# google-deepmind/mujoco_warp

Measured on NVIDIA H100. Metric: env-steps/sec (whole box) on humanoid.xml at nworld=8192 per GPU, higher is better.
Workload: dtype f32

## Files before the change

### include/mjb200.h

```cpp
#ifndef MJB200_H
#define MJB200_H

#ifdef __cplusplus
extern "C" {
#endif

typedef struct mjbModel mjbModel;
typedef struct mjbData mjbData;

mjbModel* mjb_model_create(void);
void mjb_model_destroy(mjbModel* m);
int mjb_model_set_int(mjbModel* m, const char* name, int value);
int mjb_model_set_float(mjbModel* m, const char* name, float value);
int mjb_model_set_array(mjbModel* m, const char* name, const void* dev_ptr, int nbatch);
int mjb_model_set_array_batched(mjbModel* m, const char* name, const void* dev_ptr, int nbatch, int batch_stride);
int mjb_model_finalize(mjbModel* m);

mjbData* mjb_data_create(int nworld, int nconmax, int naconmax, int njmax, int njmax_pad, int nv_pad);
void mjb_data_destroy(mjbData* d);
int mjb_data_set_array(mjbData* d, const char* name, void* dev_ptr);
int mjb_data_set_int(mjbData* d, const char* name, int value);
int mjb_data_finalize(mjbData* d, const mjbModel* m);

int mjb_step(const mjbModel* m, mjbData* d, void* stream);
// ... 7 lines not shown
int mjb_collision(const mjbModel* m, mjbData* d, void* stream);
int mjb_make_constraint(const mjbModel* m, mjbData* d, void* stream);
int mjb_fwd_velocity(const mjbModel* m, mjbData* d, void* stream);
int mjb_fwd_actuation(const mjbModel* m, mjbData* d, void* stream);
int mjb_fwd_acceleration(const mjbModel* m, mjbData* d, void* stream);
int mjb_factor_m(const mjbModel* m, mjbData* d, void* stream);
int mjb_com_vel(const mjbModel* m, mjbData* d, void* stream);
int mjb_passive(const mjbModel* m, mjbData* d, void* stream);
int mjb_rne(const mjbModel* m, mjbData* d, void* stream);
int mjb_solve_m(const mjbModel* m, mjbData* d, float* x, const float* y, void* stream);
int mjb_mul_m(const mjbModel* m, mjbData* d, float* res, const float* vec, void* stream);
int mjb_sensor_pos(const mjbModel* m, mjbData* d, void* stream);
int mjb_sensor_vel(const mjbModel* m, mjbData* d, void* stream);
int mjb_sensor_acc(const mjbModel* m, mjbData* d, void* stream);
int mjb_contact_force(const mjbModel* m, mjbData* d, const int* contact_ids, int n, int to_world_frame, float* force, void* stream);
int mjb_rungekutta4(const mjbModel* m, mjbData* d, void* stream);
int mjb_solve(const mjbModel* m, mjbData* d, void* stream);
int mjb_euler(const mjbModel* m, mjbData* d, void* stream);
int mjb_implicit(const mjbModel* m, mjbData* d, void* stream);
int mjb_ctrl_noise(const mjbModel* m, mjbData* d, const float* ctrl_center, int step, float noise_std, float noise_rate, void* stream);

int mjb_step_profile(const mjbModel* m, mjbData* d, void* stream, float* ms_out);

int mjb_last_launch_count(void);
const char* mjb_last_error(void);
const char* mjb_version(void);

#ifdef __cplusplus
}
#endif
#endif
```

### mujoco_warp_b200/__init__.py

```python

from . import scenes
from ._src import mjcf
from ._src._lib import build
from ._src.forward import camlight, collision, com_pos, crb, ctrl_noise, euler, factor_m, forward, fwd_acceleration, fwd_actuation
from ._src.forward import fwd_position, fwd_velocity, kinematics, last_launch_count, make_constraint, solve, step, step_profile, transmission
from ._src.forward import com_vel, contact_force, fwd_kinematics, get_state, implicit, mul_m, passive, rne, rungekutta4, sensor_acc, sensor_pos, sensor_vel, set_state, solve_m, step1, step2
from ._src.io import get_data_into, load_trajectory, make_data, override_model, put_data, put_model, reset_data, reset_data_keyframe
from ._src.trace import event_trace_step, flatten_trace
from ._src.types import BroadphaseFilter, BroadphaseType, ConeType, Constraint, ConstraintState, ConstraintType, Contact, Data
from ._src.types import BiasType, DynType, GainType, State, Statistic, TrnType
from ._src.types import DisableBit, EnableBit, GeomType, IntegratorType, JointType, Model, Option, OverflowType, SolverType

__all__ = [n for n in dir() if not n.startswith("_")]
```

### mujoco_warp_b200/_src/forward.py

```python

from __future__ import annotations

import torch

from . import _lib
from .types import Data, Model


def _call(name: str, m: Model, d: Data):
  if d._model is not m and d._model._handle != m._handle:
    raise ValueError("Data was created for a different Model")
  stream = torch.cuda.current_stream().cuda_stream
  _lib.check(getattr(_lib.lib(), name)(m._handle, d._handle, stream))


def step(m: Model, d: Data):
  _call("mjb_step", m, d)


def forward(m: Model, d: Data):
  _call("mjb_forward", m, d)


def fwd_position(m: Model, d: Data):
# ... 192 lines not shown
    euler(m, d)


def ctrl_noise(m: Model, d: Data, step_index: int, ctrl_center: torch.Tensor | None = None, noise_std: float = 0.01, noise_rate: float = 0.1):
  stream = torch.cuda.current_stream().cuda_stream
  ptr = ctrl_center.data_ptr() if ctrl_center is not None else None
  _lib.check(_lib.lib().mjb_ctrl_noise(m._handle, d._handle, ptr, int(step_index), float(noise_std), float(noise_rate), stream))


def last_launch_count() -> int:
  return int(_lib.lib().mjb_last_launch_count())


KERNEL_NAMES = ("position", "collision", "constraint", "velocity", "solver", "integrate")


def step_profile(m: Model, d: Data):
  import ctypes

  out = (ctypes.c_float * 6)()
  stream = torch.cuda.current_stream().cuda_stream
  _lib.check(_lib.lib().mjb_step_profile(m._handle, d._handle, stream, out))
  return dict(zip(KERNEL_NAMES, [float(x) for x in out]))
```

### mujoco_warp_b200/csrc/capi.cu

```cuda
#include <cstdio>
#include <cstdlib>
#include <algorithm>
#include <cstring>
using std::min;
#include <string>

#include "../../include/mjb200.h"
#include "mjb_types.cuh"

struct mjbModel {
  ModelDev dev;
  bool finalized;
};
struct mjbData {
  DataDev dev;
  bool finalized;
  size_t smem[6];
  cudaStream_t aux[8];
  cudaEvent_t ev_fork, ev_join[8];
  int nsplit;
  cudaStream_t sol_aux[8];
  cudaEvent_t sol_fork[8], sol_join[8];
  cudaStream_t vel_aux[8];
  cudaEvent_t vel_fork[8], vel_join[8];
// ... 126 lines not shown
  if (check(cudaMemset(d->dev.world_conadr, 0, sizeof(int) * (size_t)d->dev.nworld), "memset")) return -1;
  if (check(cudaMemset(d->dev.world_ncon, 0, sizeof(int) * (size_t)d->dev.nworld), "memset")) return -1;
  if (check(cudaMalloc(&d->dev.imp_qacc, sizeof(float) * (size_t)d->dev.nworld * (size_t)(m->dev.nv > 0 ? m->dev.nv : 1)), "cudaMalloc(imp_qacc)")) return -1;
  if (check(cudaMalloc(&d->dev.sol_list, sizeof(int) * 2 * (size_t)d->dev.nworld), "cudaMalloc(sol_list)")) return -1;
  if (check(cudaMalloc(&d->dev.sol_count, sizeof(int) * 16), "cudaMalloc(sol_count)")) return -1;
  if (check(cudaMemset(d->dev.sol_count, 0, sizeof(int) * 16), "memset")) return -1;
  for (int i = 0; i < 8; i++) {
    if (check(cudaStreamCreateWithFlags(&d->sol_aux[i], cudaStreamNonBlocking), "cudaStreamCreate")) return -1;
    if (check(cudaEventCreateWithFlags(&d->sol_fork[i], cudaEventDisableTiming), "cudaEventCreate")) return -1;
    if (check(cudaEventCreateWithFlags(&d->sol_join[i], cudaEventDisableTiming), "cudaEventCreate")) return -1;
  }
  d->dev.sol_stream = d->sol_aux[0]; d->dev.sol_fork = d->sol_fork[0]; d->dev.sol_join = d->sol_join[0];
  for (int i = 0; i < 8; i++) {
    if (check(cudaStreamCreateWithFlags(&d->vel_aux[i], cudaStreamNonBlocking), "cudaStreamCreate")) return -1;
    if (check(cudaEventCreateWithFlags(&d->vel_fork[i], cudaEventDisableTiming), "cudaEventCreate")) return -1;
    if (check(cudaEventCreateWithFlags(&d->vel_join[i], cudaEventDisableTiming), "cudaEventCreate")) return -1;
  }
  {
    const char* e = getenv("MJB_FORK");
    d->fork_velocity = (e ? atoi(e) != 0 : false) && m->dev.neq == 0 && d->dev.nworld >= 1024;
  }
  if (m->dev.integrator == INT_RK4 && !d->rk &&
      check(cudaMalloc(&d->rk, sizeof(float) * (size_t)d->dev.nworld * (size_t)(m->dev.nq + 3 * m->dev.nv + 2 * m->dev.na + 1)), "cudaMalloc(rk)")) return -1;
  d->smem[0] = smem_position(m->dev); d->smem[1] = smem_collision(m->dev, d->dev); d->smem[2] = smem_constraint(m->dev, d->dev);
  d->smem[3] = smem_velocity(m->dev); d->smem[4] = smem_solver(m->dev, d->dev); d->smem[5] = smem_integrate(m->dev);
  static const char* names[6] = {"position", "collision", "constraint", "velocity", "solver", "integrate"};
  for (int i = 0; i < 6; i++)
    if (d->smem[i] > kMaxSmem) {
      char buf[160];
      snprintf(buf, sizeof buf, "%s kernel needs %zu B of shared memory per block (> %zu): model/njmax too large for this version", names[i], d->smem[i], kMaxSmem);
      return fail(buf);
    }
  {
    const char* e = getenv("MJB_SPLIT");
    const int want = e ? atoi(e) : 2;
    if (want >= 2 && d->dev.nworld >= 1024) {
      const int ns = want > 8 ? 8 : want;
      for (int i = 0; i < ns; i++) {
        if (check(cudaStreamCreateWithFlags(&d->aux[i], cudaStreamNonBlocking), "cudaStreamCreate")) return -1;
        if (check(cudaEventCreateWithFlags(&d->ev_join[i], cudaEventDisableTiming), "cudaEventCreate")) return -1;
      }
      if (check(cudaEventCreateWithFlags(&d->ev_fork, cudaEventDisableTiming), "cudaEventCreate")) return -1;
      d->nsplit = ns;
    }
  }
  d->finalized = true;
  return 0;
}
// ... 123 lines not shown
int mjb_step_profile(const mjbModel* m, mjbData* d, void* stream, float* ms_out) {
  MJB_ENTER();
  cudaEvent_t ev[7];
  for (int i = 0; i < 7; i++) if (check(cudaEventCreate(&ev[i]), "cudaEventCreate")) return -1;
  cudaEventRecord(ev[0], s);
  MJB_LAUNCH(launch_position(m->dev, d->dev, STG_KINEMATICS | STG_COM_POS | STG_CAMLIGHT | STG_CRB | STG_TRANSMISSION, s), 1);
  cudaEventRecord(ev[1], s);
  MJB_LAUNCH(reset_contact_counters(d->dev, s), 0);
  MJB_LAUNCH(launch_collision(m->dev, d->dev, s), 1);
  cudaEventRecord(ev[2], s);
  MJB_LAUNCH(launch_constraint(m->dev, d->dev, s), 1);
  cudaEventRecord(ev[3], s);
  MJB_LAUNCH(launch_velocity(m->dev, d->dev, STG_VELOCITY | STG_ACTUATION | STG_ACCELERATION, s), 1);
  cudaEventRecord(ev[4], s);
  MJB_LAUNCH(launch_solver(m->dev, d->dev, s), 1);
  cudaEventRecord(ev[5], s);
  MJB_LAUNCH(launch_integrate(m->dev, d->dev, -1, s), 1);
  cudaEventRecord(ev[6], s);
  if (check(cudaEventSynchronize(ev[6]), "cudaEventSynchronize")) return -1;
  for (int i = 0; i < 6; i++) cudaEventElapsedTime(&ms_out[i], ev[i], ev[i + 1]);
  for (int i = 0; i < 7; i++) cudaEventDestroy(ev[i]);
  return 0;
}
int mjb_ctrl_noise(const mjbModel* m, mjbData* d, const float* ctrl_center, int step, float noise_std, float noise_rate, void* stream) {
  MJB_ENTER();
  MJB_LAUNCH(launch_ctrl_noise(m->dev, d->dev, ctrl_center, step, noise_std, noise_rate, s), 1);
  return 0;
}

}
```

### mujoco_warp_b200/csrc/k_position.cu

```cuda
#include <cstdlib>

#include "mjb_math.cuh"
#include "mjb_team.cuh"
#include "mjb_types.cuh"

namespace {

struct PosLayout {
  int qpos, xpos, xquat, xipos, xanchor, xaxis, scom, cinert, cdof, buf, arena, a_gxmat, total;
};

__host__ __device__ inline int pad4(int n) { return (n + 3) & ~3; }
__host__ __device__ inline PosLayout pos_layout(const ModelDev& m) {
  PosLayout L;
  int o = 0;
  auto take = [&](int n) { int r = o; o += pad4(n); return r; };
  L.xpos = take(3 * m.nbody); L.xquat = take(4 * m.nbody); L.xipos = take(3 * m.nbody);
  L.xanchor = take(3 * m.njnt); L.xaxis = take(3 * m.njnt);
  L.buf = L.xpos;
  if (o < pad4(6 * m.nv)) o = pad4(6 * m.nv);
  L.scom = take(3 * m.nbody); L.cinert = take(10 * m.nbody); L.cdof = take(6 * m.nv);
  L.a_gxmat = pad4(3 * m.ngeom);
  int a = pad4(9 * m.nbody);
  if (L.a_gxmat + pad4(9 * m.ngeom) > a) a = L.a_gxmat + pad4(9 * m.ngeom);
  if (pad4(m.nC) > a) a = pad4(m.nC);
  if (pad4(m.nq) > a) a = pad4(m.nq);
  L.arena = take(a);
  L.qpos = L.arena;
  L.total = o;
  return L;
}

template <int LPW, bool BAT>
__global__ void __launch_bounds__(256)
k_position(const __grid_constant__ ModelDev mp, const __grid_constant__ DataDev d, int mask) {
  extern __shared__ __align__(16) float smem[];
  constexpr int G = 32 / LPW;
  Team<LPW> T;
  T.init(d.w0, d.wn, d.nworld);
  if (T.nvalid <= 0) return;
  MJB_WORLD_MODEL(T.w)
  const int lane = T.lane, sub = T.sub, g = T.g, nval = T.nvalid;
  const bool valid = T.valid;
  const PosLayout L = pos_layout(mp);
  float* S = smem + (size_t)(threadIdx.x >> 5) * ((size_t)L.total * G + 4);
  Stager st;
  st.init(reinterpret_cast<uint64_t*>(S + (size_t)L.total * G), lane);
  const int nb = m.nbody, nj = m.njnt, ng = m.ngeom, nv = m.nv;
#define BLK(f) (S + (size_t)L.f * G)
#define ABLK(off) (S + (size_t)(L.arena + (off)) * G)
#define ROW(blk, n) ((blk) + (size_t)g * (n))
  float *qpos = ROW(BLK(qpos), m.nq), *xpos = ROW(BLK(xpos), 3 * nb), *xquat = ROW(BLK(xquat), 4 * nb), *xipos = ROW(BLK(xipos), 3 * nb),
        *xanchor = ROW(BLK(xanchor), 3 * nj), *xaxis = ROW(BLK(xaxis), 3 * nj), *scom = ROW(BLK(scom), 3 * nb), *cinert = ROW(BLK(cinert), 10 * nb),
        *cdof = ROW(BLK(cdof), 6 * nv);
  float *xmat = ROW(ABLK(0), 9 * nb), *ximat = ROW(ABLK(0), 9 * nb), *gxpos = ROW(ABLK(0), 3 * ng), *gxmat = ROW(ABLK(L.a_gxmat), 9 * ng),
        *buf = ROW(BLK(buf), 6 * nv), *Ms = ROW(ABLK(0), m.nC);
  float* crb = cinert;
  const size_t wg = (size_t)T.wg0;
#define GLOAD(blk, field, n) st.load(blk, d.field + wg * (size_t)(n), nval * (n))
#define GSTORE(field, blk, n) st.store(d.field + wg * (size_t)(n), blk, nval * (n))
  const size_t wb = (size_t)T.w;
  const bool kin = mask & STG_KINEMATICS, com = mask & STG_COM_POS, cam = mask & STG_CAMLIGHT, crbm = mask & STG_CRB;

  if (mask & (STG_KINEMATICS | STG_TRANSMISSION)) GLOAD(BLK(qpos), qpos, m.nq);
  if (!kin && (com || cam)) {
    GLOAD(BLK(xpos), xpos, 3 * nb); GLOAD(BLK(xquat), xquat, 4 * nb); GLOAD(BLK(xipos), xipos, 3 * nb);
    GLOAD(BLK(xanchor), xanchor, 3 * nj); GLOAD(BLK(xaxis), xaxis, 3 * nj);
  }
  if (!com && (cam || crbm)) { GLOAD(BLK(scom), subtree_com, 3 * nb); GLOAD(BLK(cinert), cinert, 10 * nb); GLOAD(BLK(cdof), cdof, 6 * nv); }
  st.load_wait();

  if (kin) {
    if (sub == 0) { xpos[0] = xpos[1] = xpos[2] = 0.f; xquat[0] = 1.f; xquat[1] = xquat[2] = xquat[3] = 0.f; }
    __syncwarp();
#pragma unroll 1
    for (int l = 1; l < m.nlevel; l++) {
#pragma unroll 1
      for (int i = m.level_adr[l] + sub; i < m.level_adr[l + 1]; i += LPW) {
        const int b = m.level_body[i], pid = m.body_parentid[b], jntadr = m.body_jntadr[b], jntnum = m.body_jntnum[b];
// ... 68 lines not shown
      }
    }
  }

  __syncwarp();

  if (kin) {
#pragma unroll 2
    for (int b = sub; b < nb; b += LPW) {
      q4 q = ldq(xquat + 4 * b);
      quat_to_mat(q, xmat + 9 * b);
      st3(xipos + 3 * b, ld3(xpos + 3 * b) + qrot(q, ld3(m.body_ipos + 3 * b)));
    }
#pragma unroll 1
    for (int s = valid ? sub : m.nsite; s < m.nsite; s += LPW) {
      const int b = m.site_bodyid[s];
      q4 q = ldq(xquat + 4 * b);
      float mat[9];
      st3(d.site_xpos + (wb * m.nsite + s) * 3, ld3(xpos + 3 * b) + qrot(q, ld3(m.site_pos + 3 * s)));
      quat_to_mat(qmul(q, ldq(m.site_quat + 4 * s)), mat);
      for (int k = 0; k < 9; k++) d.site_xmat[(wb * m.nsite + s) * 9 + k] = mat[k];
    }
    st.store_fence();
    GSTORE(xpos, BLK(xpos), 3 * nb); GSTORE(xquat, BLK(xquat), 4 * nb); GSTORE(xmat, ABLK(0), 9 * nb); GSTORE(xipos, BLK(xipos), 3 * nb);
    GSTORE(xanchor, BLK(xanchor), 3 * nj); GSTORE(xaxis, BLK(xaxis), 3 * nj);
    st.store_commit();
    if (!com) {
      st.store_wait_read();
#pragma unroll 2
      for (int b = sub; b < nb; b += LPW) quat_to_mat(qmul(ldq(xquat + 4 * b), ldq(m.body_iquat + 4 * b)), ximat + 9 * b);
      st.store_fence();
      GSTORE(ximat, ABLK(0), 9 * nb);
      st.store_commit();
    }
  }
  __syncwarp();

  if (com) {
#pragma unroll 2
    for (int b = sub; b < nb; b += LPW) st3(scom + 3 * b, ld3(xipos + 3 * b) * m.body_mass[b]);
    __syncwarp();
#pragma unroll 1
    for (int l = m.nlevel - 2; l >= 0; l--) {
#pragma unroll 1
      for (int i = m.level_adr[l] + sub; i < m.level_adr[l + 1]; i += LPW) {
        const int b = m.level_body[i];
        v3 acc = ld3(scom + 3 * b);
        for (int c = m.body_childadr[b]; c < m.body_childadr[b + 1]; c++) acc = acc + ld3(scom + 3 * m.body_childid[c]);
        st3(scom + 3 * b, acc);
      }
      __syncwarp();
    }
#pragma unroll 2
    for (int b = sub; b < nb; b += LPW) {
      const float ms = m.body_subtreemass[b];
// ... 26 lines not shown
      int dof = m.jnt_dofadr[j];
      const v3 offset = ld3(scom + 3 * m.body_rootid[b]) - ld3(xanchor + 3 * j);
      if (t == JNT_FREE || t == JNT_BALL) {
        float xm[9];
        quat_to_mat(ldq(xquat + 4 * b), xm);
        if (t == JNT_FREE) {
          for (int k = 0; k < 18; k++) cdof[6 * dof + k] = 0.f;
          cdof[6 * dof + 3] = 1.f; cdof[6 * (dof + 1) + 4] = 1.f; cdof[6 * (dof + 2) + 5] = 1.f;
          dof += 3;
        }
        for (int k = 0; k < 3; k++) {
          v3 col = matcol(xm, k);
          st3(cdof + 6 * (dof + k), col); st3(cdof + 6 * (dof + k) + 3, cross(col, offset));
        }
      } else if (t == JNT_SLIDE) {
        st3(cdof + 6 * dof, mk3(0.f, 0.f, 0.f)); st3(cdof + 6 * dof + 3, ld3(xaxis + 3 * j));
      } else {
        v3 ax = ld3(xaxis + 3 * j);
        st3(cdof + 6 * dof, ax); st3(cdof + 6 * dof + 3, cross(ax, offset));
      }
    }
    st.store_fence();
    GSTORE(subtree_com, BLK(scom), 3 * nb); GSTORE(cinert, BLK(cinert), 10 * nb); GSTORE(cdof, BLK(cdof), 6 * nv);
    if (kin) GSTORE(ximat, ABLK(0), 9 * nb);
    st.store_commit();
  }
  __syncwarp();

  if (mask & STG_CAMLIGHT) {
#pragma unroll 1
    for (int c = valid ? sub : m.ncam; c < m.ncam; c += LPW) {
      const int mode = m.cam_mode[c], b = m.cam_bodyid[c], tb = m.cam_targetbodyid[c];
      const bool is_target = mode == CAM_TARGETBODY || mode == CAM_TARGETBODYCOM;
      v3 p; float mat[9];
      if (mode == CAM_TRACK) {
        for (int k = 0; k < 9; k++) mat[k] = m.cam_mat0[9 * c + k];
        p = ld3(xpos + 3 * b) + ld3(m.cam_pos0 + 3 * c);
      } else if (mode == CAM_TRACKCOM) {
        for (int k = 0; k < 9; k++) mat[k] = m.cam_mat0[9 * c + k];
        p = ld3(scom + 3 * b) + ld3(m.cam_poscom0 + 3 * c);
      } else if (is_target && tb >= 0) {
        q4 q = ldq(xquat + 4 * b);
        p = ld3(xpos + 3 * b) + qrot(q, ld3(m.cam_pos + 3 * c));
        v3 tp = mode == CAM_TARGETBODYCOM ? ld3(scom + 3 * tb) : ld3(xpos + 3 * tb);
        v3 m3 = normalize(p - tp), m1 = normalize(cross(mk3(0.f, 0.f, 1.f), m3)), m2 = normalize(cross(m3, m1));
        mat[0] = m1.x; mat[1] = m2.x; mat[2] = m3.x; mat[3] = m1.y; mat[4] = m2.y; mat[5] = m3.y; mat[6] = m1.z; mat[7] = m2.z; mat[8] = m3.z;
      } else {
// ... 26 lines not shown
      }
      if (norm) dir = normalize(dir);
      st3(d.light_xpos + (wb * m.nlight + l) * 3, p);
      st3(d.light_xdir + (wb * m.nlight + l) * 3, dir);
    }
  }


  if (kin) {
    st.store_wait_read();
#pragma unroll 2
    for (int gi = sub; gi < ng; gi += LPW) {
      const int b = m.geom_bodyid[gi];
      if (m.body_weldid[b] == 0 && (m.nmocap == 0 || m.body_mocapid[m.body_rootid[b]] == -1)) {
        for (int k = 0; k < 3; k++) gxpos[3 * gi + k] = d.geom_xpos[(wb * ng + gi) * 3 + k];
        for (int k = 0; k < 9; k++) gxmat[9 * gi + k] = d.geom_xmat[(wb * ng + gi) * 9 + k];
      } else {
        q4 q = ldq(xquat + 4 * b);
        st3(gxpos + 3 * gi, ld3(xpos + 3 * b) + qrot(q, ld3(m.geom_pos + 3 * gi)));
        quat_to_mat(qmul(q, ldq(m.geom_quat + 4 * gi)), gxmat + 9 * gi);
      }
    }
    st.store_fence();
    GSTORE(geom_xpos, ABLK(0), 3 * ng); GSTORE(geom_xmat, ABLK(L.a_gxmat), 9 * ng);
    st.store_commit();
  }

  if (crbm) {
    st.store_wait_read();
#pragma unroll 1
    for (int l = m.nlevel - 2; l >= 1; l--) {
#pragma unroll 1
      for (int i = m.level_adr[l] + sub; i < m.level_adr[l + 1]; i += LPW) {
        const int b = m.level_body[i];
        float acc[10];
#pragma unroll
        for (int k = 0; k < 10; k++) acc[k] = crb[10 * b + k];
#pragma unroll 1
        for (int c = m.body_childadr[b]; c < m.body_childadr[b + 1]; c++) {
          const float* cc = crb + 10 * m.body_childid[c];
#pragma unroll
          for (int k = 0; k < 10; k++) acc[k] += cc[k];
        }
#pragma unroll
        for (int k = 0; k < 10; k++) crb[10 * b + k] = acc[k];
      }
      __syncwarp();
    }
#pragma unroll 2
    for (int dd = sub; dd < nv; dd += LPW) inert_vec(crb + 10 * m.dof_bodyid[dd], cdof + 6 * dd, buf + 6 * dd);
    __syncwarp();
#pragma unroll 4
    for (int e = sub; e < m.nC; e += LPW) {
      const int i = m.M_entry_row[e], j = m.M_colind[e];
      float v = dot6(cdof + 6 * j, buf + 6 * i);
      if (i == j) v += m.dof_armature[i];
      Ms[e] = v;
    }
    st.store_fence();
    GSTORE(crb, BLK(cinert), 10 * nb); GSTORE(M, ABLK(0), m.nC);
    st.store_commit();
  }
  st.store_wait_read();
#undef GLOAD
#undef GSTORE
#undef BLK
#undef ABLK
#undef ROW
}

}

static TeamShape pos_shape(const ModelDev& m) {
  TeamShape t = team_shape((size_t)pos_layout(m).total, "MJB_LPW_POS", "MJB_WPB_POS");
  if (m.batched && t.lpw != 32) { t = team_shape_fixed((size_t)pos_layout(m).total, 32, 2); }
  return t;
}
size_t smem_position(const ModelDev& m) { return pos_shape(m).block_bytes; }

cudaError_t launch_position(const ModelDev& m, const DataDev& d, int mask, cudaStream_t s) {
  const TeamShape t = pos_shape(m);
  const size_t smem = t.block_bytes;
  const int lpw = t.lpw, G = 32 / lpw, wpb = t.wpb;
  void (*kern)(ModelDev, DataDev, int) = m.batched ? k_position<32, true> : lpw == 4 ? k_position<4, false> : lpw == 8 ? k_position<8, false> : lpw == 16 ? k_position<16, false> : k_position<32, false>;
  static size_t configured[5] = {0, 0, 0, 0, 0};
  const int ki = m.batched ? 4 : lpw == 4 ? 0 : lpw == 8 ? 1 : lpw == 16 ? 2 : 3;
  if (smem > 48 * 1024 && smem > configured[ki]) {
    cudaError_t e = cudaFuncSetAttribute(kern, cudaFuncAttributeMaxDynamicSharedMemorySize, (int)smem);
    if (e != cudaSuccess) return e;
    configured[ki] = smem;
  }
  const int ngroups = (d.wn + G - 1) / G, grid = (ngroups + wpb - 1) / wpb;
  kern<<<grid, 32 * wpb, smem, s>>>(m, d, mask);
  return cudaGetLastError();
}
```

### mujoco_warp_b200/csrc/k_velocity.cu

```cuda
#include <cstdlib>

#include "mjb_math.cuh"
#include "mjb_team.cuh"
#include "mjb_types.cuh"

namespace {

struct VelLayout { int qvel, cdof, cinert, cvel, cdofdot, cacc, cfrc, qpas, qbias, qact, qsm, qld, x, af, total; };
__host__ __device__ inline VelLayout vel_layout(const ModelDev& m) {
  VelLayout L;
  int o = 0;
  auto take = [&](int n) { int r = o; o += (n + 3) & ~3; return r; };
  L.qvel = take(m.nv);
  const int a0 = o;
  L.cdof = take(6 * m.nv); L.cinert = take(10 * m.nbody); L.cvel = take(6 * m.nbody);
  L.cdofdot = take(6 * m.nv); L.cacc = take(6 * m.nbody); L.cfrc = take(6 * m.nbody);
  L.qld = a0;
  if (o - a0 < ((m.qld_total + 3) & ~3)) o = a0 + ((m.qld_total + 3) & ~3);
  L.qpas = take(m.nv); L.qbias = take(m.nv); L.qact = take(m.nv); L.qsm = take(m.nv);
  L.x = L.qpas; L.af = take(m.nu);
  L.total = o;
  return L;
}

template <int LPW>
__device__ __forceinline__ void team_chol_upper(float* U, int n, float* x, bool solve, int sub) {
#pragma unroll 1
  for (int j = 0; j < n; j++) {
    const int iend = solve ? n + 1 : n;
#pragma unroll 1
    for (int i = j + sub; i < iend; i += LPW) {
      const bool rhs = i == n;
      const float* col = rhs ? x : U + i;
      const int cs = rhs ? 1 : n;
      float s0 = rhs ? x[j] : U[j * n + i], s1 = 0.f;
      int k = 0;
#pragma unroll 4
      for (; k + 1 < j; k += 2) {
        s0 -= U[k * n + j] * col[k * cs];
        s1 -= U[(k + 1) * n + j] * col[(k + 1) * cs];
      }
      if (k < j) s0 -= U[k * n + j] * col[k * cs];
      if (rhs) x[j] = s0 + s1; else U[j * n + i] = s0 + s1;
// ... 196 lines not shown
    if (v_all || (mask & STG_RNE)) {
    for (int k = sub; k < 6; k += LPW) cacc[k] = k < 3 ? 0.f : ((m.disableflags & DSBL_GRAVITY) ? 0.f : -(k == 3 ? m.gravity_x : k == 4 ? m.gravity_y : m.gravity_z));
    __syncwarp();
#pragma unroll 1
    for (int l = 1; l < m.nlevel; l++) {
#pragma unroll 1
      for (int i = m.level_adr[l] + sub; i < m.level_adr[l + 1]; i += LPW) {
        const int b = m.level_body[i], pid = m.body_parentid[b];
        float a[6];
#pragma unroll
        for (int k = 0; k < 6; k++) a[k] = cacc[6 * pid + k];
#pragma unroll 1
        for (int q = 0; q < m.body_dofnum[b]; q++) {
          const int dof = m.body_dofadr[b] + q;
          const float v = qvel[dof];
#pragma unroll
          for (int k = 0; k < 6; k++) a[k] += cdofdot[6 * dof + k] * v;
        }
#pragma unroll
        for (int k = 0; k < 6; k++) cacc[6 * b + k] = a[k];
      }
      __syncwarp();
    }
#pragma unroll 2
    for (int b = sub; b < nb; b += LPW) {
      float f[6] = {0.f, 0.f, 0.f, 0.f, 0.f, 0.f};
      if (b > 0) {
        float iv[6], g[6];
        inert_vec(cinert + 10 * b, cacc + 6 * b, f);
        inert_vec(cinert + 10 * b, cvel + 6 * b, iv);
        motion_cross_force(cvel + 6 * b, iv, g);
#pragma unroll
        for (int k = 0; k < 6; k++) f[k] += g[k];
      }
#pragma unroll
      for (int k = 0; k < 6; k++) cfrc[6 * b + k] = f[k];
    }
    __syncwarp();
#pragma unroll 1
    for (int l = m.nlevel - 2; l >= 0; l--) {
#pragma unroll 1
      for (int i = m.level_adr[l] + sub; i < m.level_adr[l + 1]; i += LPW) {
        const int b = m.level_body[i];
        float acc[6];
#pragma unroll
        for (int k = 0; k < 6; k++) acc[k] = cfrc[6 * b + k];
// ... 134 lines not shown
#pragma unroll
      for (int k = 0; k < MREG; k++) {
        const int e = sub + k * LPW;
        if (e >= e0 && e < e1) U[(m.M_colind[e] - start) * n + (m.M_entry_row[e] - start)] = mreg[k];
      }
#pragma unroll 1
      for (int e = max(e0, MREG * LPW) + ((sub - max(e0, MREG * LPW)) % LPW + LPW) % LPW; e < e1; e += LPW)
        U[(m.M_colind[e] - start) * n + (m.M_entry_row[e] - start)] = Mw[e];
      __syncwarp();
      team_chol_upper<LPW>(U, n, x + start, acc, sub);
    }
    st.store_fence();
    if (acc) { GSTORE(qfrc_smooth, qsm, nv); GSTORE(qacc_smooth, x, nv); }
    GSTORE(qLD, qld, m.qld_total);
    st.store_commit();
  }
  st.store_wait_read();
#undef GLOAD
#undef GSTORE
}

}

static TeamShape vel_shape(const ModelDev& m) {
  TeamShape t = team_shape((size_t)vel_layout(m).total, "MJB_LPW_VEL", "MJB_WPB_VEL");
  if (m.batched && t.lpw != 32) t = team_shape_fixed((size_t)vel_layout(m).total, 32, 2);
  return t;
}
size_t smem_velocity(const ModelDev& m) { return vel_shape(m).block_bytes; }

template <bool PEXT>
static void (*vel_kernel(int lpw, bool bat))(ModelDev, DataDev, int) {
  if (bat) return k_velocity<PEXT, 32, true>;
  return lpw == 4 ? k_velocity<PEXT, 4, false> : lpw == 8 ? k_velocity<PEXT, 8, false> : lpw == 16 ? k_velocity<PEXT, 16, false> : k_velocity<PEXT, 32, false>;
}

cudaError_t launch_velocity(const ModelDev& m, const DataDev& d, int mask, cudaStream_t s) {
  const TeamShape t = vel_shape(m);
  const size_t smem = t.block_bytes;
  static size_t configured[2][5] = {{0, 0, 0, 0, 0}, {0, 0, 0, 0, 0}};
  const int ext = (m.has_gravcomp || m.ntendon > 0) ? 1 : 0;
  const int lpw = t.lpw, G = 32 / lpw, wpb = t.wpb, ki = m.batched ? 4 : lpw == 4 ? 0 : lpw == 8 ? 1 : lpw == 16 ? 2 : 3;
  void (*kern)(ModelDev, DataDev, int) = ext ? vel_kernel<true>(lpw, m.batched) : vel_kernel<false>(lpw, m.batched);
  if (smem > 48 * 1024 && smem > configured[ext][ki]) {
    cudaError_t e = cudaFuncSetAttribute(kern, cudaFuncAttributeMaxDynamicSharedMemorySize, (int)smem);
    if (e != cudaSuccess) return e;
    configured[ext][ki] = smem;
  }
  const int ngroups = (d.wn + G - 1) / G, grid = (ngroups + wpb - 1) / wpb;
  kern<<<grid, 32 * wpb, smem, s>>>(m, d, mask);
  return cudaGetLastError();
}
```

### mujoco_warp_b200/csrc/mjb_team.cuh

```cuda
#pragma once
#include <cstdint>
#include <cstdlib>
#include <cuda_runtime.h>

#include "mjb_math.cuh"

template <int LPW>
__device__ __forceinline__ float team_sum(float v) {
#pragma unroll
  for (int o = LPW / 2; o > 0; o >>= 1) v += __shfl_xor_sync(FULL_MASK, v, o);
  return v;
}
template <int LPW>
__device__ __forceinline__ int team_sum_i(int v) {
#pragma unroll
  for (int o = LPW / 2; o > 0; o >>= 1) v += __shfl_xor_sync(FULL_MASK, v, o);
  return v;
}
template <int LPW>
__device__ __forceinline__ bool team_any(bool p, int g) {
  const unsigned b = __ballot_sync(FULL_MASK, p);
  return LPW == 32 ? b != 0u : ((b >> (g * LPW)) & ((1u << (LPW & 31)) - 1u)) != 0u;
}

// ... 43 lines not shown
    asm volatile("fence.proxy.async.shared::cta;" ::: "memory");
    __syncwarp();
  }
  __device__ __forceinline__ void store(float* g, const float* s, int n) {
    if (bulk_ok(g, s, n)) {
      if (lane == 0) {
        asm volatile("cp.async.bulk.global.shared::cta.bulk_group [%0], [%1], %2;" ::"l"(g), "r"(smem_u32(s)), "r"((uint32_t)n * 4u) : "memory");
        pending_store = true;
      }
    } else {
#pragma unroll 1
      for (int i = lane; i < n; i += 32) g[i] = s[i];
    }
  }
  __device__ __forceinline__ void store_commit() {
    if (lane == 0 && pending_store) asm volatile("cp.async.bulk.commit_group;" ::: "memory");
  }
  __device__ __forceinline__ void store_wait_read() {
    if (lane == 0 && pending_store) { asm volatile("cp.async.bulk.wait_group.read 0;" ::: "memory"); pending_store = false; }
    __syncwarp();
  }
};

struct TeamShape { int lpw, wpb; size_t warp_bytes, block_bytes; };
inline TeamShape team_shape(size_t world_words, const char* env_lpw, const char* env_wpb) {
  constexpr size_t kBlockMax = 200 * 1024;
  auto bytes = [&](int lpw) { return (world_words * (size_t)(32 / lpw) + 4) * sizeof(float); };
  const char* e = getenv(env_lpw);
  int lpw = e ? atoi(e) : 8;
  if (lpw != 4 && lpw != 8 && lpw != 16 && lpw != 32) lpw = 8;
  while (lpw < 32 && bytes(lpw) > kBlockMax / 2) lpw *= 2;
  e = getenv(env_wpb);
  int wpb = e ? atoi(e) : 2;
  if (wpb < 1) wpb = 1;
  if (wpb > 8) wpb = 8;
  while (wpb > 1 && bytes(lpw) * wpb > kBlockMax) wpb--;
  TeamShape t;
  t.lpw = lpw; t.wpb = wpb; t.warp_bytes = bytes(lpw); t.block_bytes = t.warp_bytes * wpb;
  return t;
}

inline TeamShape team_shape_fixed(size_t world_words, int lpw, int wpb) {
  TeamShape t;
  t.lpw = lpw; t.wpb = wpb; t.warp_bytes = (world_words * (size_t)(32 / lpw) + 4) * sizeof(float);
  while (t.wpb > 1 && t.warp_bytes * t.wpb > 200 * 1024) t.wpb--;
  t.block_bytes = t.warp_bytes * t.wpb;
  return t;
}

template <int LPW>
struct Team {
  static constexpr int G = 32 / LPW;
  int lane, sub, g;
  int wg0, nvalid;
  int w;
  bool valid;
// ... 10 lines not shown
```

### mujoco_warp_b200/csrc/mjb_types.cuh

```cuda
#pragma once
#include <cuda_runtime.h>

#define MJB_MODEL_INTS(X) \
  X(nq) X(nv) X(nu) X(nbody) X(njnt) X(ngeom) X(nsite) X(ncam) X(nlight) X(nC) X(ntree) X(nJmom) X(nlevel) \
  X(nxn_npair) X(nlimit) X(nfricdof) X(nmaxpyramid) X(integrator) X(cone) X(solver) X(iterations) \
  X(ls_iterations) X(disableflags) X(enableflags) X(broadphase) X(broadphase_filter) X(qld_total) X(maxtree) X(has_multicontact_geom) X(neq) X(nlimit_ball) X(has_gravcomp) X(nmocap) X(npair) X(has_convex_pair) X(ccd_iterations) X(epa_iterations) X(nsensor) X(nsensordata) X(sensor_subtree_vel) X(sensor_rne_postconstraint) X(nmesh) X(na) X(ntendon) X(nJten) X(ntenfric) X(nwrap)
#define MJB_MODEL_FLOATS(X) \
  X(timestep) X(tolerance) X(ls_tolerance) X(impratio_invsqrt) X(meaninertia) X(gravity_x) X(gravity_y) X(gravity_z) X(ccd_tolerance)
#define MJB_MODEL_IARRS(X) \
  X(body_parentid) X(body_rootid) X(body_weldid) X(body_mocapid) X(body_jntnum) X(body_jntadr) X(body_dofnum) X(body_dofadr) \
  X(body_childadr) X(body_childid) X(level_adr) X(level_body) \
  X(jnt_type) X(jnt_qposadr) X(jnt_dofadr) X(jnt_bodyid) X(jnt_actfrclimited) X(jnt_actgravcomp) X(jnt_limited_adr) \
  X(dof_bodyid) X(dof_jntid) X(dof_parentid) X(dof_fricloss_adr) X(M_rownnz) X(M_rowadr) X(M_colind) X(M_entry_row) X(mulm_rowadr) X(mulm_col) X(mulm_madr) \
  X(tree_dofadr) X(tree_dofnum) X(tree_qLDadr) \
  X(geom_type) X(geom_condim) X(geom_bodyid) X(geom_priority) \
  X(actuator_trnid) X(actuator_gaintype) X(actuator_biastype) X(actuator_ctrllimited) X(actuator_forcelimited) \
  X(actuator_dyntype) X(actuator_actadr) X(actuator_actnum) X(actuator_actlimited) X(actuator_actearly) X(actuator_trntype) \
  X(ten_J_rownnz) X(ten_J_rowadr) X(ten_J_colind) X(tendon_adr) X(tendon_num) X(wrap_objid) X(tendon_limited) X(tendon_actfrclimited) \
  X(moment_rownnz0) X(moment_rowadr0) X(moment_colind0) X(dofact_adr) X(dofact_act) X(dofact_mom) \
  X(cam_mode) X(cam_bodyid) X(cam_targetbodyid) X(light_mode) X(light_bodyid) X(light_targetbodyid) X(site_bodyid) \
  X(nxn_geom_pair) X(nxn_pairid) X(body_isdofancestor) X(eq_type) X(eq_obj1id) X(eq_obj2id) X(jnt_limited_ball_adr) X(pair_dim) \
  X(sensor_type) X(sensor_datatype) X(sensor_needstage) X(sensor_objtype) X(sensor_objid) X(sensor_reftype) X(sensor_refid) X(sensor_dim) X(sensor_adr) X(site_type) \
  X(geom_dataid) X(mesh_vertadr) X(mesh_vertnum) X(mesh_graphadr) X(mesh_graph) X(mesh_polynum) X(mesh_polyadr) X(mesh_polyvertadr) X(mesh_polyvertnum) \
  X(mesh_polyvert) X(mesh_polymapadr) X(mesh_polymapnum) X(mesh_polymap)
// ... 117 lines not shown
       STG_COMVEL = 16, STG_PASSIVE = 32, STG_RNE = 64 };

constexpr int MJB_WARPS_PER_BLOCK = 1;

cudaError_t launch_position(const ModelDev& m, const DataDev& d, int stage_mask, cudaStream_t s);
cudaError_t launch_collision(const ModelDev& m, const DataDev& d, cudaStream_t s);
cudaError_t launch_collision_mesh(const ModelDev& m, const DataDev& d, cudaStream_t s);
size_t smem_collision_mesh(const ModelDev& m, const DataDev& d);
cudaError_t reset_contact_counters(const DataDev& d, cudaStream_t s);
cudaError_t launch_constraint(const ModelDev& m, const DataDev& d, cudaStream_t s);
cudaError_t launch_efc_csr(const ModelDev& m, const DataDev& d, cudaStream_t s);
cudaError_t launch_velocity(const ModelDev& m, const DataDev& d, int stage_mask, cudaStream_t s);
cudaError_t launch_solve_m(const ModelDev& m, const DataDev& d, float* x, const float* y, cudaStream_t s);
cudaError_t launch_mul_m(const ModelDev& m, const DataDev& d, float* res, const float* vec, cudaStream_t s);
cudaError_t launch_solver(const ModelDev& m, const DataDev& d, cudaStream_t s);
int solver_launch_count(const ModelDev& m, const DataDev& d);
cudaError_t launch_integrate(const ModelDev& m, const DataDev& d, int integrator, cudaStream_t s);
cudaError_t launch_implicit_solve(const ModelDev& m, const DataDev& d, float* qacc_out, cudaStream_t s);
size_t smem_implicit(const ModelDev& m);
cudaError_t launch_sensor(const ModelDev& m, const DataDev& d, int stages, cudaStream_t s);
cudaError_t launch_contact_force(const ModelDev& m, const DataDev& d, const int* contact_ids, int n, int to_world, float* out, cudaStream_t s);
cudaError_t launch_rk_stage(const ModelDev& m, const DataDev& d, float* rk, int stage, cudaStream_t s);
cudaError_t launch_ctrl_noise(const ModelDev& m, const DataDev& d, const float* ctrl_center, int step, float std, float rate, cudaStream_t s);
size_t smem_position(const ModelDev& m);
size_t smem_collision(const ModelDev& m, const DataDev& d);
size_t smem_constraint(const ModelDev& m, const DataDev& d);
size_t smem_velocity(const ModelDev& m);
size_t smem_solver(const ModelDev& m, const DataDev& d);
size_t smem_integrate(const ModelDev& m);
```

Before: 19.41 million.

## Shrink position/velocity smem layouts and pick warps-per-block from occupancy model

Repacks the shared-memory layouts of the position and velocity kernels so more buffers alias each other, which shrinks the per-world footprint. Warps-per-block is now chosen automatically by modelling SM residency from shared memory, register and block limits against nworld, and the shared-memory carveout is set explicitly. The goal is more worlds resident per SM and fewer launch waves. Adds a residency query API and an extra store_wait_read to protect against the new aliasing, at the risk of hazards if any aliased buffer is still live.

After: 20.80 million (median of 6 runs). +7.2%, better.

```diff
diff --git a/include/mjb200.h b/include/mjb200.h
--- a/include/mjb200.h
+++ b/include/mjb200.h
@@ -53,6 +53,8 @@
 
 int mjb_step_profile(const mjbModel* m, mjbData* d, void* stream, float* ms_out);
 
+int mjb_team_residency(const mjbModel* m, const mjbData* d, int* position_worlds, int* velocity_worlds);
+
 int mjb_last_launch_count(void);
 const char* mjb_last_error(void);
 const char* mjb_version(void);
diff --git a/mujoco_warp_b200/__init__.py b/mujoco_warp_b200/__init__.py
--- a/mujoco_warp_b200/__init__.py
+++ b/mujoco_warp_b200/__init__.py
@@ -3,7 +3,7 @@
 from ._src import mjcf
 from ._src._lib import build
 from ._src.forward import camlight, collision, com_pos, crb, ctrl_noise, euler, factor_m, forward, fwd_acceleration, fwd_actuation
-from ._src.forward import fwd_position, fwd_velocity, kinematics, last_launch_count, make_constraint, solve, step, step_profile, transmission
+from ._src.forward import fwd_position, fwd_velocity, kinematics, last_launch_count, make_constraint, solve, step, step_profile, team_residency, transmission
 from ._src.forward import com_vel, contact_force, fwd_kinematics, get_state, implicit, mul_m, passive, rne, rungekutta4, sensor_acc, sensor_pos, sensor_vel, set_state, solve_m, step1, step2
 from ._src.io import get_data_into, load_trajectory, make_data, override_model, put_data, put_model, reset_data, reset_data_keyframe
 from ._src.trace import event_trace_step, flatten_trace
diff --git a/mujoco_warp_b200/_src/forward.py b/mujoco_warp_b200/_src/forward.py
--- a/mujoco_warp_b200/_src/forward.py
+++ b/mujoco_warp_b200/_src/forward.py
@@ -238,3 +238,13 @@
   stream = torch.cuda.current_stream().cuda_stream
   _lib.check(_lib.lib().mjb_step_profile(m._handle, d._handle, stream, out))
   return dict(zip(KERNEL_NAMES, [float(x) for x in out]))
+
+
+def team_residency(m: Model, d: Data):
+  import ctypes
+
+  f = _lib.lib().mjb_team_residency
+  f.argtypes = [ctypes.c_void_p, ctypes.c_void_p, ctypes.POINTER(ctypes.c_int), ctypes.POINTER(ctypes.c_int)]
+  pos, vel = ctypes.c_int(), ctypes.c_int()
+  _lib.check(f(m._handle, d._handle, ctypes.byref(pos), ctypes.byref(vel)))
+  return {"position": pos.value, "velocity": vel.value}
diff --git a/mujoco_warp_b200/csrc/capi.cu b/mujoco_warp_b200/csrc/capi.cu
--- a/mujoco_warp_b200/csrc/capi.cu
+++ b/mujoco_warp_b200/csrc/capi.cu
@@ -172,8 +172,8 @@
   }
   if (m->dev.integrator == INT_RK4 && !d->rk &&
       check(cudaMalloc(&d->rk, sizeof(float) * (size_t)d->dev.nworld * (size_t)(m->dev.nq + 3 * m->dev.nv + 2 * m->dev.na + 1)), "cudaMalloc(rk)")) return -1;
-  d->smem[0] = smem_position(m->dev); d->smem[1] = smem_collision(m->dev, d->dev); d->smem[2] = smem_constraint(m->dev, d->dev);
-  d->smem[3] = smem_velocity(m->dev); d->smem[4] = smem_solver(m->dev, d->dev); d->smem[5] = smem_integrate(m->dev);
+  d->smem[0] = smem_position(m->dev, d->dev); d->smem[1] = smem_collision(m->dev, d->dev); d->smem[2] = smem_constraint(m->dev, d->dev);
+  d->smem[3] = smem_velocity(m->dev, d->dev); d->smem[4] = smem_solver(m->dev, d->dev); d->smem[5] = smem_integrate(m->dev);
   static const char* names[6] = {"position", "collision", "constraint", "velocity", "solver", "integrate"};
   for (int i = 0; i < 6; i++)
     if (d->smem[i] > kMaxSmem) {
@@ -343,6 +343,13 @@
   for (int i = 0; i < 7; i++) cudaEventDestroy(ev[i]);
   return 0;
 }
+int mjb_team_residency(const mjbModel* m, const mjbData* d, int* position_worlds, int* velocity_worlds) {
+  if (!m || !d || !m->finalized || !d->finalized) return fail("model/data not finalized");
+  if (!position_worlds || !velocity_worlds) return fail("mjb_team_residency: null output");
+  if (check(resident_worlds_position(m->dev, d->dev, position_worlds), "resident_worlds_position")) return -1;
+  if (check(resident_worlds_velocity(m->dev, d->dev, velocity_worlds), "resident_worlds_velocity")) return -1;
+  return 0;
+}
 int mjb_ctrl_noise(const mjbModel* m, mjbData* d, const float* ctrl_center, int step, float noise_std, float noise_rate, void* stream) {
   MJB_ENTER();
   MJB_LAUNCH(launch_ctrl_noise(m->dev, d->dev, ctrl_center, step, noise_std, noise_rate, s), 1);
diff --git a/mujoco_warp_b200/csrc/k_position.cu b/mujoco_warp_b200/csrc/k_position.cu
--- a/mujoco_warp_b200/csrc/k_position.cu
+++ b/mujoco_warp_b200/csrc/k_position.cu
@@ -7,7 +7,7 @@
 namespace {
 
 struct PosLayout {
-  int qpos, xpos, xquat, xipos, xanchor, xaxis, scom, cinert, cdof, buf, arena, a_gxmat, total;
+  int qpos, xpos, xquat, xipos, xanchor, xaxis, scom, cinert, cdof, buf, arena, gxpos, gxmat, M, total;
 };
 
 __host__ __device__ inline int pad4(int n) { return (n + 3) & ~3; }
@@ -16,17 +16,14 @@
   int o = 0;
   auto take = [&](int n) { int r = o; o += pad4(n); return r; };
   L.xpos = take(3 * m.nbody); L.xquat = take(4 * m.nbody); L.xipos = take(3 * m.nbody);
-  L.xanchor = take(3 * m.njnt); L.xaxis = take(3 * m.njnt);
-  L.buf = L.xpos;
-  if (o < pad4(6 * m.nv)) o = pad4(6 * m.nv);
-  L.scom = take(3 * m.nbody); L.cinert = take(10 * m.nbody); L.cdof = take(6 * m.nv);
-  L.a_gxmat = pad4(3 * m.ngeom);
-  int a = pad4(9 * m.nbody);
-  if (L.a_gxmat + pad4(9 * m.ngeom) > a) a = L.a_gxmat + pad4(9 * m.ngeom);
-  if (pad4(m.nC) > a) a = pad4(m.nC);
-  if (pad4(m.nq) > a) a = pad4(m.nq);
-  L.arena = take(a);
+  L.xanchor = take(3 * m.njnt); L.xaxis = take(3 * m.njnt); L.scom = take(3 * m.nbody);
+  L.arena = take(pad4(m.nq) > pad4(9 * m.nbody) ? m.nq : 9 * m.nbody);
   L.qpos = L.arena;
+  L.gxpos = L.xipos; L.gxmat = L.gxpos + pad4(3 * m.ngeom);
+  L.buf = L.xpos; L.M = L.buf + pad4(6 * m.nv);
+  if (o < L.gxmat + pad4(9 * m.ngeom)) o = L.gxmat + pad4(9 * m.ngeom);
+  if (o < L.M + pad4(m.nC)) o = L.M + pad4(m.nC);
+  L.cinert = take(10 * m.nbody); L.cdof = take(6 * m.nv);
   L.total = o;
   return L;
 }
@@ -48,13 +45,12 @@
   st.init(reinterpret_cast<uint64_t*>(S + (size_t)L.total * G), lane);
   const int nb = m.nbody, nj = m.njnt, ng = m.ngeom, nv = m.nv;
 #define BLK(f) (S + (size_t)L.f * G)
-#define ABLK(off) (S + (size_t)(L.arena + (off)) * G)
 #define ROW(blk, n) ((blk) + (size_t)g * (n))
   float *qpos = ROW(BLK(qpos), m.nq), *xpos = ROW(BLK(xpos), 3 * nb), *xquat = ROW(BLK(xquat), 4 * nb), *xipos = ROW(BLK(xipos), 3 * nb),
         *xanchor = ROW(BLK(xanchor), 3 * nj), *xaxis = ROW(BLK(xaxis), 3 * nj), *scom = ROW(BLK(scom), 3 * nb), *cinert = ROW(BLK(cinert), 10 * nb),
         *cdof = ROW(BLK(cdof), 6 * nv);
-  float *xmat = ROW(ABLK(0), 9 * nb), *ximat = ROW(ABLK(0), 9 * nb), *gxpos = ROW(ABLK(0), 3 * ng), *gxmat = ROW(ABLK(L.a_gxmat), 9 * ng),
-        *buf = ROW(BLK(buf), 6 * nv), *Ms = ROW(ABLK(0), m.nC);
+  float *xmat = ROW(BLK(arena), 9 * nb), *ximat = ROW(BLK(arena), 9 * nb), *gxpos = ROW(BLK(gxpos), 3 * ng), *gxmat = ROW(BLK(gxmat), 9 * ng),
+        *buf = ROW(BLK(buf), 6 * nv), *Ms = ROW(BLK(M), m.nC);
   float* crb = cinert;
   const size_t wg = (size_t)T.wg0;
 #define GLOAD(blk, field, n) st.load(blk, d.field + wg * (size_t)(n), nval * (n))
@@ -169,7 +165,7 @@
       for (int k = 0; k < 9; k++) d.site_xmat[(wb * m.nsite + s) * 9 + k] = mat[k];
     }
     st.store_fence();
-    GSTORE(xpos, BLK(xpos), 3 * nb); GSTORE(xquat, BLK(xquat), 4 * nb); GSTORE(xmat, ABLK(0), 9 * nb); GSTORE(xipos, BLK(xipos), 3 * nb);
+    GSTORE(xpos, BLK(xpos), 3 * nb); GSTORE(xquat, BLK(xquat), 4 * nb); GSTORE(xmat, BLK(arena), 9 * nb); GSTORE(xipos, BLK(xipos), 3 * nb);
     GSTORE(xanchor, BLK(xanchor), 3 * nj); GSTORE(xaxis, BLK(xaxis), 3 * nj);
     st.store_commit();
     if (!com) {
@@ -177,7 +173,7 @@
 #pragma unroll 2
       for (int b = sub; b < nb; b += LPW) quat_to_mat(qmul(ldq(xquat + 4 * b), ldq(m.body_iquat + 4 * b)), ximat + 9 * b);
       st.store_fence();
-      GSTORE(ximat, ABLK(0), 9 * nb);
+      GSTORE(ximat, BLK(arena), 9 * nb);
       st.store_commit();
     }
   }
@@ -250,7 +246,7 @@
     }
     st.store_fence();
     GSTORE(subtree_com, BLK(scom), 3 * nb); GSTORE(cinert, BLK(cinert), 10 * nb); GSTORE(cdof, BLK(cdof), 6 * nv);
-    if (kin) GSTORE(ximat, ABLK(0), 9 * nb);
+    if (kin) GSTORE(ximat, BLK(arena), 9 * nb);
     st.store_commit();
   }
   __syncwarp();
@@ -323,7 +319,7 @@
       }
     }
     st.store_fence();
-    GSTORE(geom_xpos, ABLK(0), 3 * ng); GSTORE(geom_xmat, ABLK(L.a_gxmat), 9 * ng);
+    GSTORE(geom_xpos, BLK(gxpos), 3 * ng); GSTORE(geom_xmat, BLK(gxmat), 9 * ng);
     st.store_commit();
   }
 
@@ -359,39 +355,52 @@
       Ms[e] = v;
     }
     st.store_fence();
-    GSTORE(crb, BLK(cinert), 10 * nb); GSTORE(M, ABLK(0), m.nC);
+    GSTORE(crb, BLK(cinert), 10 * nb); GSTORE(M, BLK(M), m.nC);
     st.store_commit();
   }
   st.store_wait_read();
 #undef GLOAD
 #undef GSTORE
 #undef BLK
-#undef ABLK
 #undef ROW
 }
 
 }
 
-static TeamShape pos_shape(const ModelDev& m) {
-  TeamShape t = team_shape((size_t)pos_layout(m).total, "MJB_LPW_POS", "MJB_WPB_POS");
+static void (*pos_kernel(const ModelDev& m, int lpw))(ModelDev, DataDev, int) {
+  return m.batched ? k_position<32, true> : lpw == 4 ? k_position<4, false> : lpw == 8 ? k_position<8, false> : lpw == 16 ? k_position<16, false> : k_position<32, false>;
+}
+
+static TeamShape pos_shape(const ModelDev& m, const DataDev& d) {
+  TeamShape t = team_shape((size_t)pos_layout(m).total, d.wn, "MJB_LPW_POS", "MJB_WPB_POS", [&](int lpw) { return kernel_regs(pos_kernel(m, lpw)); });
   if (m.batched && t.lpw != 32) { t = team_shape_fixed((size_t)pos_layout(m).total, 32, 2); }
   return t;
 }
-size_t smem_position(const ModelDev& m) { return pos_shape(m).block_bytes; }
+size_t smem_position(const ModelDev& m, const DataDev& d) { return pos_shape(m, d).block_bytes; }
+
+static cudaError_t pos_configured(const ModelDev& m, const TeamShape& t, void (**kern)(ModelDev, DataDev, int)) {
+  static TeamConfig configured[5];
+  const int lpw = t.lpw, ki = m.batched ? 4 : lpw == 4 ? 0 : lpw == 8 ? 1 : lpw == 16 ? 2 : 3;
+  *kern = pos_kernel(m, lpw);
+  return team_configure(*kern, t.block_bytes, &configured[ki]);
+}
 
 cudaError_t launch_position(const ModelDev& m, const DataDev& d, int mask, cudaStream_t s) {
-  const TeamShape t = pos_shape(m);
-  const size_t smem = t.block_bytes;
-  const int lpw = t.lpw, G = 32 / lpw, wpb = t.wpb;
-  void (*kern)(ModelDev, DataDev, int) = m.batched ? k_position<32, true> : lpw == 4 ? k_position<4, false> : lpw == 8 ? k_position<8, false> : lpw == 16 ? k_position<16, false> : k_position<32, false>;
-  static size_t configured[5] = {0, 0, 0, 0, 0};
-  const int ki = m.batched ? 4 : lpw == 4 ? 0 : lpw == 8 ? 1 : lpw == 16 ? 2 : 3;
-  if (smem > 48 * 1024 && smem > configured[ki]) {
-    cudaError_t e = cudaFuncSetAttribute(kern, cudaFuncAttributeMaxDynamicSharedMemorySize, (int)smem);
-    if (e != cudaSuccess) return e;
-    configured[ki] = smem;
-  }
-  const int ngroups = (d.wn + G - 1) / G, grid = (ngroups + wpb - 1) / wpb;
-  kern<<<grid, 32 * wpb, smem, s>>>(m, d, mask);
+  const TeamShape t = pos_shape(m, d);
+  void (*kern)(ModelDev, DataDev, int);
+  cudaError_t e = pos_configured(m, t, &kern);
+  if (e != cudaSuccess) return e;
+  const int G = 32 / t.lpw, ngroups = (d.wn + G - 1) / G, grid = (ngroups + t.wpb - 1) / t.wpb;
+  kern<<<grid, 32 * t.wpb, t.block_bytes, s>>>(m, d, mask);
   return cudaGetLastError();
 }
+
+cudaError_t resident_worlds_position(const ModelDev& m, const DataDev& d, int* worlds) {
+  const TeamShape t = pos_shape(m, d);
+  void (*kern)(ModelDev, DataDev, int);
+  int blocks = 0;
+  cudaError_t e = pos_configured(m, t, &kern);
+  if (e == cudaSuccess) e = cudaOccupancyMaxActiveBlocksPerMultiprocessor(&blocks, kern, 32 * t.wpb, t.block_bytes);
+  *worlds = blocks * t.wpb * (32 / t.lpw);
+  return e;
+}
diff --git a/mujoco_warp_b200/csrc/k_velocity.cu b/mujoco_warp_b200/csrc/k_velocity.cu
--- a/mujoco_warp_b200/csrc/k_velocity.cu
+++ b/mujoco_warp_b200/csrc/k_velocity.cu
@@ -10,15 +10,18 @@
 __host__ __device__ inline VelLayout vel_layout(const ModelDev& m) {
   VelLayout L;
   int o = 0;
-  auto take = [&](int n) { int r = o; o += (n + 3) & ~3; return r; };
-  L.qvel = take(m.nv);
+  auto pad = [](int n) { return (n + 3) & ~3; };
+  auto take = [&](int n) { int r = o; o += pad(n); return r; };
+  L.qpas = take(m.nv); L.qbias = take(m.nv);
+  L.qsm = L.qpas; L.x = L.qbias;
   const int a0 = o;
-  L.cdof = take(6 * m.nv); L.cinert = take(10 * m.nbody); L.cvel = take(6 * m.nbody);
-  L.cdofdot = take(6 * m.nv); L.cacc = take(6 * m.nbody); L.cfrc = take(6 * m.nbody);
+  L.cdof = take(6 * m.nv); L.cinert = take(10 * m.nbody); L.qvel = take(m.nv);
+  L.cvel = take(6 * m.nbody); L.cdofdot = take(6 * (m.nv > m.nbody ? m.nv : m.nbody)); L.cacc = take(6 * m.nbody);
+  L.cfrc = L.cdofdot;
+  if (pad(m.nv) + pad(m.nu) <= L.cvel - L.cinert) { L.qact = L.cinert; L.af = L.cinert + pad(m.nv); }
+  else { L.qact = take(m.nv); L.af = take(m.nu); }
   L.qld = a0;
-  if (o - a0 < ((m.qld_total + 3) & ~3)) o = a0 + ((m.qld_total + 3) & ~3);
-  L.qpas = take(m.nv); L.qbias = take(m.nv); L.qact = take(m.nv); L.qsm = take(m.nv);
-  L.x = L.qpas; L.af = take(m.nu);
+  if (o - a0 < pad(m.qld_total)) o = a0 + pad(m.qld_total);
   L.total = o;
   return L;
 }
@@ -261,6 +264,7 @@
       }
       __syncwarp();
     }
+    st.store_wait_read();
 #pragma unroll 2
     for (int b = sub; b < nb; b += LPW) {
       float f[6] = {0.f, 0.f, 0.f, 0.f, 0.f, 0.f};
@@ -441,32 +445,46 @@
 
 }
 
-static TeamShape vel_shape(const ModelDev& m) {
-  TeamShape t = team_shape((size_t)vel_layout(m).total, "MJB_LPW_VEL", "MJB_WPB_VEL");
-  if (m.batched && t.lpw != 32) t = team_shape_fixed((size_t)vel_layout(m).total, 32, 2);
-  return t;
-}
-size_t smem_velocity(const ModelDev& m) { return vel_shape(m).block_bytes; }
-
 template <bool PEXT>
 static void (*vel_kernel(int lpw, bool bat))(ModelDev, DataDev, int) {
   if (bat) return k_velocity<PEXT, 32, true>;
   return lpw == 4 ? k_velocity<PEXT, 4, false> : lpw == 8 ? k_velocity<PEXT, 8, false> : lpw == 16 ? k_velocity<PEXT, 16, false> : k_velocity<PEXT, 32, false>;
 }
+static bool vel_ext(const ModelDev& m) { return m.has_gravcomp || m.ntendon > 0; }
+static void (*vel_kernel(const ModelDev& m, int lpw))(ModelDev, DataDev, int) {
+  return vel_ext(m) ? vel_kernel<true>(lpw, m.batched) : vel_kernel<false>(lpw, m.batched);
+}
+
+static TeamShape vel_shape(const ModelDev& m, const DataDev& d) {
+  TeamShape t = team_shape((size_t)vel_layout(m).total, d.wn, "MJB_LPW_VEL", "MJB_WPB_VEL", [&](int lpw) { return kernel_regs(vel_kernel(m, lpw)); });
+  if (m.batched && t.lpw != 32) t = team_shape_fixed((size_t)vel_layout(m).total, 32, 2);
+  return t;
+}
+size_t smem_velocity(const ModelDev& m, const DataDev& d) { return vel_shape(m, d).block_bytes; }
+
+static cudaError_t vel_configured(const ModelDev& m, const TeamShape& t, void (**kern)(ModelDev, DataDev, int)) {
+  static TeamConfig configured[2][5];
+  const int ext = vel_ext(m) ? 1 : 0, ki = m.batched ? 4 : t.lpw == 4 ? 0 : t.lpw == 8 ? 1 : t.lpw == 16 ? 2 : 3;
+  *kern = vel_kernel(m, t.lpw);
+  return team_configure(*kern, t.block_bytes, &configured[ext][ki]);
+}
 
 cudaError_t launch_velocity(const ModelDev& m, const DataDev& d, int mask, cudaStream_t s) {
-  const TeamShape t = vel_shape(m);
-  const size_t smem = t.block_bytes;
-  static size_t configured[2][5] = {{0, 0, 0, 0, 0}, {0, 0, 0, 0, 0}};
-  const int ext = (m.has_gravcomp || m.ntendon > 0) ? 1 : 0;
-  const int lpw = t.lpw, G = 32 / lpw, wpb = t.wpb, ki = m.batched ? 4 : lpw == 4 ? 0 : lpw == 8 ? 1 : lpw == 16 ? 2 : 3;
-  void (*kern)(ModelDev, DataDev, int) = ext ? vel_kernel<true>(lpw, m.batched) : vel_kernel<false>(lpw, m.batched);
-  if (smem > 48 * 1024 && smem > configured[ext][ki]) {
-    cudaError_t e = cudaFuncSetAttribute(kern, cudaFuncAttributeMaxDynamicSharedMemorySize, (int)smem);
-    if (e != cudaSuccess) return e;
-    configured[ext][ki] = smem;
-  }
-  const int ngroups = (d.wn + G - 1) / G, grid = (ngroups + wpb - 1) / wpb;
-  kern<<<grid, 32 * wpb, smem, s>>>(m, d, mask);
+  const TeamShape t = vel_shape(m, d);
+  void (*kern)(ModelDev, DataDev, int);
+  cudaError_t e = vel_configured(m, t, &kern);
+  if (e != cudaSuccess) return e;
+  const int G = 32 / t.lpw, ngroups = (d.wn + G - 1) / G, grid = (ngroups + t.wpb - 1) / t.wpb;
+  kern<<<grid, 32 * t.wpb, t.block_bytes, s>>>(m, d, mask);
   return cudaGetLastError();
 }
+
+cudaError_t resident_worlds_velocity(const ModelDev& m, const DataDev& d, int* worlds) {
+  const TeamShape t = vel_shape(m, d);
+  void (*kern)(ModelDev, DataDev, int);
+  int blocks = 0;
+  cudaError_t e = vel_configured(m, t, &kern);
+  if (e == cudaSuccess) e = cudaOccupancyMaxActiveBlocksPerMultiprocessor(&blocks, kern, 32 * t.wpb, t.block_bytes);
+  *worlds = blocks * t.wpb * (32 / t.lpw);
+  return e;
+}
diff --git a/mujoco_warp_b200/csrc/mjb_team.cuh b/mujoco_warp_b200/csrc/mjb_team.cuh
--- a/mujoco_warp_b200/csrc/mjb_team.cuh
+++ b/mujoco_warp_b200/csrc/mjb_team.cuh
@@ -1,4 +1,6 @@
 #pragma once
+#include <algorithm>
+#include <climits>
 #include <cstdint>
 #include <cstdlib>
 #include <cuda_runtime.h>
@@ -89,8 +91,51 @@
   }
 };
 
+struct SmLimits { int sms; size_t smem_per_sm, reserved_per_block; int blocks, warps, regs; };
+inline const SmLimits& sm_limits() {
+  static const SmLimits l = [] {
+    int dev = 0, sms = 0, smem = 0, reserved = 0, blocks = 0, threads = 0, regs = 0;
+    cudaGetDevice(&dev);
+    cudaDeviceGetAttribute(&sms, cudaDevAttrMultiProcessorCount, dev);
+    cudaDeviceGetAttribute(&smem, cudaDevAttrMaxSharedMemoryPerMultiprocessor, dev);
+    cudaDeviceGetAttribute(&reserved, cudaDevAttrReservedSharedMemoryPerBlock, dev);
+    cudaDeviceGetAttribute(&blocks, cudaDevAttrMaxBlocksPerMultiprocessor, dev);
+    cudaDeviceGetAttribute(&threads, cudaDevAttrMaxThreadsPerMultiProcessor, dev);
+    cudaDeviceGetAttribute(&regs, cudaDevAttrMaxRegistersPerMultiprocessor, dev);
+    return SmLimits{sms, (size_t)smem, (size_t)reserved, blocks, threads / 32, regs};
+  }();
+  return l;
+}
+
+template <class K>
+inline int kernel_regs(K* kern) {
+  cudaFuncAttributes a;
+  return cudaFuncGetAttributes(&a, kern) == cudaSuccess ? a.numRegs : 0;
+}
+
+inline size_t sm_block_bytes(size_t bytes) { return ((bytes + 127) & ~(size_t)127) + sm_limits().reserved_per_block; }
+
+struct TeamConfig { size_t smem = 0; int carveout = -1; };
+template <class K>
+inline cudaError_t team_configure(K* kern, size_t smem, TeamConfig* c) {
+  const size_t per_sm = sm_limits().smem_per_sm, block = sm_block_bytes(smem), fit = per_sm / block;
+  const size_t pct = fit > 0 ? (100 * fit * block + per_sm - 1) / per_sm : 100;
+  const int carveout = pct < 100 ? (int)pct : (int)cudaSharedmemCarveoutMaxShared;
+  cudaError_t e = cudaSuccess;
+  if (carveout != c->carveout) {
+    e = cudaFuncSetAttribute(kern, cudaFuncAttributePreferredSharedMemoryCarveout, carveout);
+    if (e == cudaSuccess) c->carveout = carveout;
+  }
+  if (e == cudaSuccess && smem > 48 * 1024 && smem > c->smem) {
+    e = cudaFuncSetAttribute(kern, cudaFuncAttributeMaxDynamicSharedMemorySize, (int)smem);
+    if (e == cudaSuccess) c->smem = smem;
+  }
+  return e;
+}
+
 struct TeamShape { int lpw, wpb; size_t warp_bytes, block_bytes; };
-inline TeamShape team_shape(size_t world_words, const char* env_lpw, const char* env_wpb) {
+template <class F>
+inline TeamShape team_shape(size_t world_words, int nworld, const char* env_lpw, const char* env_wpb, F regs_of) {
   constexpr size_t kBlockMax = 200 * 1024;
   auto bytes = [&](int lpw) { return (world_words * (size_t)(32 / lpw) + 4) * sizeof(float); };
   const char* e = getenv(env_lpw);
@@ -98,7 +143,23 @@
   if (lpw != 4 && lpw != 8 && lpw != 16 && lpw != 32) lpw = 8;
   while (lpw < 32 && bytes(lpw) > kBlockMax / 2) lpw *= 2;
   e = getenv(env_wpb);
-  int wpb = e ? atoi(e) : 2;
+  int wpb = 2;
+  if (e) {
+    wpb = atoi(e);
+  } else {
+    const SmLimits& sm = sm_limits();
+    const long groups = (nworld + 32 / lpw - 1) / (32 / lpw);
+    const int warp_regs = (regs_of(lpw) * 32 + 255) & ~255;
+    auto rounds = [&](int w) {
+      long per_sm = (long)(sm.smem_per_sm / sm_block_bytes(bytes(lpw) * w));
+      per_sm = std::min({per_sm, (long)sm.blocks, (long)(sm.warps / w)});
+      if (warp_regs > 0) per_sm = std::min(per_sm, (long)(sm.regs / warp_regs / w));
+      const long fit = per_sm * sm.sms, blocks = (groups + w - 1) / w;
+      return fit > 0 ? (blocks + fit - 1) / fit : LONG_MAX;
+    };
+    for (int w : {1, 4})
+      if (bytes(lpw) * w <= kBlockMax && rounds(w) < rounds(wpb)) wpb = w;
+  }
   if (wpb < 1) wpb = 1;
   if (wpb > 8) wpb = 8;
   while (wpb > 1 && bytes(lpw) * wpb > kBlockMax) wpb--;
diff --git a/mujoco_warp_b200/csrc/mjb_types.cuh b/mujoco_warp_b200/csrc/mjb_types.cuh
--- a/mujoco_warp_b200/csrc/mjb_types.cuh
+++ b/mujoco_warp_b200/csrc/mjb_types.cuh
@@ -163,9 +163,11 @@
 cudaError_t launch_contact_force(const ModelDev& m, const DataDev& d, const int* contact_ids, int n, int to_world, float* out, cudaStream_t s);
 cudaError_t launch_rk_stage(const ModelDev& m, const DataDev& d, float* rk, int stage, cudaStream_t s);
 cudaError_t launch_ctrl_noise(const ModelDev& m, const DataDev& d, const float* ctrl_center, int step, float std, float rate, cudaStream_t s);
-size_t smem_position(const ModelDev& m);
+size_t smem_position(const ModelDev& m, const DataDev& d);
 size_t smem_collision(const ModelDev& m, const DataDev& d);
 size_t smem_constraint(const ModelDev& m, const DataDev& d);
-size_t smem_velocity(const ModelDev& m);
+size_t smem_velocity(const ModelDev& m, const DataDev& d);
+cudaError_t resident_worlds_position(const ModelDev& m, const DataDev& d, int* worlds);
+cudaError_t resident_worlds_velocity(const ModelDev& m, const DataDev& d, int* worlds);
 size_t smem_solver(const ModelDev& m, const DataDev& d);
 size_t smem_integrate(const ModelDev& m);
```
